# Hippogriff/prifit

Hardware: AMD Instinct MI355X
Metric: shapes/sec (fwd+bwd) B=24x2048 pts, PointNet++-MSG+ellipsoid fit (higher is better)
Workload: dtype f32; 1 GPU; configs[2]: PointNet++-MSG + mean-shift(10 it, <=25 clusters) + ellipsoid fit + convex loss, B=24x2048 per GPU, fwd+bwd+Adam; global_batch=24, points=2048, parallelism=dp1, cloud=blobs, embedding=clustered, backbone_grad_param=sa1.conv_blocks.0.0.weight, launch=eager

## Files before the change

### include/prifit_hip.h

```cpp
#ifndef PRIFIT_HIP_H
#define PRIFIT_HIP_H

#include <stdint.h>

#ifdef __cplusplus
extern "C" {
#endif

#define PRIFIT_OK 0
#define PRIFIT_EINVAL (-1)
#define PRIFIT_ELAUNCH (-2)

#define PRIFIT_ABI_VERSION 700
int prifit_version(const char **arch);


int prifit_fps(const float *xyz, int B, int N, int npoint, const int64_t *start_idx,
               int64_t *out_idx, float *new_xyz, void *stream);

int prifit_ball_query(const float *xyz, const float *new_xyz, int B, int N, int S, int R,
                      const float *radius2, const int *nsample, void *const *out, int idx64,
                      void *stream);

int prifit_three_nn(const float *xyz1, const float *xyz2, int B, int N, int S, int32_t *idx,
                    float *dist, float *weight, void *stream);

int prifit_square_distance(const float *src, const float *dst, int B, int S, int N, float *out,
                           void *stream);


int prifit_group_gather(const float *feat, const float *xyz, const float *new_xyz,
                        const int32_t *idx, int B, int N, int S, int K, int C, int order,
                        int ld_out, float *out, void *stream);

int prifit_group_scatter_add(const float *gout, int ld_gout, int col0, const int32_t *idx, int B,
                             int N, int S, int K, int C, float *dfeat, void *stream);

int prifit_pack_cols(const float *w, int rows, int src_cols, const int32_t *map, int dst_cols, float *out, void *stream);
int prifit_unpack_cols(const float *g, int rows, int dst_cols, const int32_t *inv_off, const int32_t *inv_idx, int src_cols,
                       float *gw, void *stream);
int prifit_pack_cols_max_jobs(void);
int prifit_pack_cols_multi(int njobs, const float *const *w, const int32_t *rows, const int32_t *src_cols, const int32_t *const *map,
                           const int32_t *dst_cols, float *const *out, void *stream);
int prifit_unpack_cols_multi(int njobs, const float *const *g, const int32_t *rows, const int32_t *dst_cols, const int32_t *const *inv_off,
                             const int32_t *const *inv_idx, const int32_t *src_cols, float *const *gw, void *stream);

int prifit_three_interpolate(const float *points2, const int32_t *idx, const float *weight, int B,
                             int N, int S, int C, int ld_out, int col0, float *out, void *stream);

int prifit_three_interpolate_bwd(const float *gout, int ld_gout, int col0, const int32_t *idx,
                                 const float *weight, int B, int N, int S, int C, float *dpoints2,
                                 void *stream);
int prifit_fp_rows(const float *points2, const int32_t *idx, const float *weight, const float *points1, int B, int N, int S, int D2,
                   int D1, int kp, float *out, void *stream);


#define PRIFIT_GEMM_NT 0
#define PRIFIT_GEMM_NN 1
#define PRIFIT_GEMM_TN 2
#define PRIFIT_EPI_NONE 0
#define PRIFIT_EPI_CHORD 1
#define PRIFIT_EPI_MSKERNEL 2
#define PRIFIT_EPI_MSBWD 3

int prifit_gemm_f32(int layout, int M, int N, int K, const float *A, long long lda, long long strideA,
                    const float *B, long long ldb, long long strideB, float *C, long long ldc,
                    long long strideC, int batch, int splitk, const float *a_scale,
                    const float *a_shift, const float *b_scale, const float *b_shift,
                    const float *bias, long long bias_batch_stride, float *col_stats, int epilogue,
                    const float *epi_batch_scalar, const float *epi_aux, long long ld_aux,
                    long long stride_aux, const float *epi_row_add, float *a_rowsum, int accumulate, void *stream);

int prifit_chord_sym_f32(const float *A, long long lda, long long strideA, float *C, long long ldc, long long strideC,
                         int n, int K, int batch, unsigned long long *owner_key, void *stream);
int prifit_chord_sym_mask(const float *A, long long lda, long long strideA, const float *thr, uint32_t *mask, int n, int K, int batch,
                          unsigned long long *owner_key, void *stream);
int prifit_gram_sym_f32(const float *A, long long lda, long long strideA, float *C, long long ldc, long long strideC, int n, int K,
                        int batch, void *stream);

int prifit_gemm_pool_f32(int M, int N, int K, const float *A, long long lda, const float *W, long long ldb, float *Y,
                         long long ldc, const float *a_scale, const float *a_shift, const float *bias, float *col_stats,
                         float *cand, void *stream);
int prifit_gemm_pool_supported(int M, int N, int K);

int prifit_gemm_stream_f32(int layout, int M, int N, int K, const float *A, long long lda, const float *B,
                           long long ldb, float *C, long long ldc, const float *a_scale, const float *a_shift,
                           const float *bias, float *col_stats, void *stream);
int prifit_gemm_stream_supported(int layout, int M, int N, int K);
int prifit_gemm_stream_slabs(int M, int K);

int prifit_gemm_dual_nn_f32(int M, int N, int K1, int K2, const float *A1, const float *A2, long long lda,
                            long long strideA, const float *B1, const float *B2, long long ldb, long long strideB,
                            float *C, long long ldc, long long strideC, int batch, int splitk, int accumulate,
                            void *stream);

int prifit_gemm_dgrad_bnred_f32(int M, int N, int K, const float *dY, long long lda, const float *W, long long ldb,
                                float *G, long long ldc, const float *Yprev, long long ldy, const float *scale,
                                const float *shift, const float *mean, const float *invstd, float *red_slab, void *stream);
int prifit_slab_sum(const float *part, int nslab, long long n, float *out, void *stream);
int prifit_global_pool_winners_supported(int Cout, int Cin);
int prifit_global_pool_winners_f32(int Bs, int K, int Cout, int Cin, const int32_t *arg, const float *T, const float *W,
                                   long long ldw, const float *X, long long ldx, float *dX, long long lddx, float *dW,
                                   long long lddw, void *stream);

int prifit_gemm_stream_gather_f32(int M, int N, const int32_t *idx, const float *U, const float *Vc, int n_points, int n_centres,
                                  int rows_per_centre, const float *B, long long ldb, float *C, long long ldc,
                                  const float *a_scale, const float *a_shift, const float *bias, float *col_stats, void *stream);
int prifit_gemm_stream_bwd_gather_f32(long long P, int Cout, const float *G, const float *Y, const float *scale,
                                      const float *shift, const float *coef_a, const float *coef_b, const float *coef_d,
                                      const float *W, long long ldw, const int32_t *idx, const float *U, const float *Vc,
                                      int n_points, int n_centres, int rows_per_centre, const float *p_scale,
                                      const float *p_shift, const float *p_mean, const float *p_invstd, float *Gp, long long ldgp,
                                      float *red_slab, float *dW, long long lddw, float *workspace, void *stream);
int prifit_gemm_stream_pool_f32(int M, int N, int K, const float *A, long long lda, const float *B, long long ldb,
                                float *C, long long ldc, const float *a_scale, const float *a_shift, const float *bias,
                                float *col_stats, float *cand, void *stream);
int prifit_pool_from_candidates(const float *cand, const float *scale, const float *shift, int G, int K, int C,
                                int rows_per_sample, float slope, float *out, long long ldo, int32_t *arg, float *ystar,
                                void *stream);

int prifit_gemm_stream_dgrad_f32(int M, int N, int K, const float *dY, long long lda, const float *W, long long ldb,
                                 float *G, long long ldc, const float *Yprev, long long ldy, const float *scale,
                                 const float *shift, const float *mean, const float *invstd, float *red_slab, void *stream);

int prifit_pool_bwd_table(const float *gp, long long ldgp, const float *Y, long long ldy, const int32_t *arg,
                          const float *scale, const float *shift, const float *coef_a, int G, int K, int C, float slope,
                          float *T, void *stream);
int prifit_gemm_stream_dgrad_pool_f32(int M, int N, int K, const float *Y, long long lda, const float *W, long long ldb,
                                      float *G, long long ldc, const float *bias_dW, const int32_t *pool_arg,
                                      const float *pool_T, const float *coef_b, int pool_K, const float *Yprev,
                                      long long ldy, const float *scale, const float *shift, const float *mean,
                                      const float *invstd, float *red_slab, void *stream);
int prifit_gemm_stream_tn_pool_f32(int Mo, int No, long long P, const float *Y, long long ldy, const float *A,
                                   long long lda, float *out, long long ldo, const float *b_scale,
                                   const float *b_shift, const int32_t *pool_arg, const float *pool_T,
                                   const float *coef_b, const float *coef_d, int pool_K, float *workspace,
                                   void *stream);

int prifit_gemm_stream_tn_bn_f32(int Mo, int No, long long P, const float *G, const float *Y, long long ldy, const float *A,
                                 long long lda, float *out, long long ldo, const float *b_scale, const float *b_shift,
                                 const float *scale, const float *shift, const float *coef_a, const float *coef_b,
                                 const float *coef_d, float *workspace, void *stream);
int prifit_gemm_stream_dgrad_bn_f32(int M, int N, int K, const float *Gin, const float *Y, long long lda, const float *W,
                                    long long ldb, float *G, long long ldc, const float *scale_l, const float *shift_l,
                                    const float *coef_a, const float *coef_b, const float *coef_d, const float *Yprev,
                                    long long ldy, const float *scale, const float *shift, const float *mean,
                                    const float *invstd, float *red_slab, void *stream);
int prifit_gemm_stream_tn_f32(int Mo, int No, long long P, const float *G, long long ldg, const float *A,
                              long long lda, float *out, long long ldo, const float *b_scale,
                              const float *b_shift, float *workspace, void *stream);
long long prifit_gemm_stream_tn_workspace(int Mo, int No, long long P);
int prifit_gemm_stream_tn_supported(int Mo, int No, long long P);

int prifit_gemm_tile_m(int N);
// ... 326 lines not shown
```

### prifit_amd/csrc/gemm.hip

```cpp
#include <stdlib.h>

#include <type_traits>

#include "common.h"

typedef float f32x16 __attribute__((ext_vector_type(16)));

enum { LAY_NT = 0, LAY_NN = 1, LAY_TN = 2 };
enum { EPI_NONE = 0, EPI_CHORD = 1, EPI_MSKERNEL = 2, EPI_MSBWD = 3, EPI_BNRED = 4 };

struct GemmArgs {
    const float *A, *B;
    float *C;
    int M, N, K;
    long long lda, ldb, ldc;
    long long sA, sB, sC;
    int batch, splitk;
    const float *a_scale, *a_shift;
    const float *b_scale, *b_shift;
    const float *bias;
    long long bias_stride;
    float *stats;
    int epi;
    const float *epi_batch_scalar;
    const float *aux;
    const float *row_add;
    float *a_rowsum;
    long long ldaux, sAux;
    const float *red_scale, *red_shift, *red_mean, *red_invstd;
    long long dA2, dB2;
    int kswitch;
    int accumulate;
    int vecA, vecB;
    int ntiles;
    float *cand;
};

#ifndef GEMM_W8
#define GEMM_W8 6
#endif
constexpr int BK = 32;
constexpr int PAD = 4;

__device__ __forceinline__ float4 ld4(const float *p) { return *reinterpret_cast<const float4 *>(p); }

template <int ROWS, bool KC, bool VEC, bool AFF, int NTH>
struct TileLoader {
    static constexpr int NV = ROWS * BK / 4 / NTH;
    static_assert(NV * NTH * 4 == ROWS * BK, "tile must divide evenly over the threads");
    float4 v[NV];
    const float *ptr[NV];
    int klo[NV];
    int c0[NV];
    unsigned okmask[NV];
    long long step;
    int K, R, cclamp;

    __device__ __forceinline__ void init(const float *__restrict__ base, long long ld, int r0, int R_, int K_)
    {
        K = K_; R = R_;
        step = KC ? (long long)BK : (long long)BK * ld;
#pragma unroll
        for (int p = 0; p < NV; ++p) {
            const int id = threadIdx.x + NTH * p;
            if (KC) {
                const int gr = r0 + id / (BK / 4);
                klo[p] = (id % (BK / 4)) * 4;
                okmask[p] = gr < R ? 0xFu : 0u;
                ptr[p] = base + (long long)(gr < R ? gr : 0) * ld + (klo[p] < K ? klo[p] : 0);
                c0[p] = 0;
            } else {
                klo[p] = id / (ROWS / 4);
                const int gr = r0 + (id % (ROWS / 4)) * 4;
                unsigned m = 0;
#pragma unroll
                for (int j = 0; j < 4; ++j) m |= (gr + j < R) ? (1u << j) : 0u;
                okmask[p] = m;
                c0[p] = m ? gr : 0;
                ptr[p] = base + (long long)klo[p] * ld + c0[p];
            }
        }
    }

    int kload;
// ... 163 lines not shown
    int klo[NV], c0[NV];
    __amdgpu_buffer_rsrc_t rs;
    const float *base;
    int step4, K, kload;

    __device__ __forceinline__ void init(const float *__restrict__ b, long long ld, int r0, int R, int K_)
    {
        K = K_;
        base = b;
        rs = __builtin_amdgcn_make_buffer_rsrc(const_cast<float *>(b), 0, 0x7ffffffc, 0x00020000);
        step4 = KC ? BK * 4 : (int)(BK * ld * 4);
#pragma unroll
        for (int p = 0; p < NV; ++p) {
            const int id = threadIdx.x + NTH * p;
            if (KC) {
                const int row = r0 + id / (BK / 4);
                klo[p] = (id % (BK / 4)) * 4;
                c0[p] = 0;
                voff[p] = row < R ? (int)(((long long)row * ld + klo[p]) * 4) : OOBV;
            } else {
                klo[p] = id / (ROWS / 4);
                c0[p] = r0 + (id % (ROWS / 4)) * 4;
                voff[p] = c0[p] < R ? (int)(((long long)klo[p] * ld + c0[p]) * 4) : OOBV;
                if (c0[p] >= R) c0[p] = 0;
            }
        }
    }
    __device__ __forceinline__ void load(int k0, const float *__restrict__, const float *__restrict__) { load(k0); }
    __device__ __forceinline__ void shift(long long delta)
    {
        base += delta;
        rs = __builtin_amdgcn_make_buffer_rsrc(const_cast<float *>(base), 0, 0x7ffffffc, 0x00020000);
    }
    __device__ __forceinline__ void load(int k0)
    {
        kload = k0;
        const int soff = (k0 / BK) * step4;
        if (k0 + BK <= K) {
#pragma unroll
            for (int p = 0; p < NV; ++p) {
                const f32x4v t = __builtin_bit_cast(f32x4v, __builtin_amdgcn_raw_buffer_load_b128(rs, voff[p], soff, 0));
                v[p] = make_float4(t.x, t.y, t.z, t.w);
            }
        } else {
#pragma unroll
            for (int p = 0; p < NV; ++p) {
                const int vo = k0 + klo[p] < K ? voff[p] : OOBV;
                const f32x4v t = __builtin_bit_cast(f32x4v, __builtin_amdgcn_raw_buffer_load_b128(rs, vo, soff, 0));
                v[p] = make_float4(t.x, t.y, t.z, t.w);
            }
        }
    }
    __device__ __forceinline__ void finish(const float *__restrict__ scale, const float *__restrict__ shift)
    {
        if (!AFF) return;
#pragma unroll
        for (int p = 0; p < NV; ++p) {
            const int gk = kload + klo[p];
            const bool ok = voff[p] != OOBV && gk < K;
            const int cc = KC ? (gk < K ? gk : 0) : c0[p];
            const float4 s = ld4(scale + cc), t = ld4(shift + cc);
            float4 x = v[p];
            x.x = fmaxf(fmaf(x.x, s.x, t.x), 0.f); x.y = fmaxf(fmaf(x.y, s.y, t.y), 0.f);
            x.z = fmaxf(fmaf(x.z, s.z, t.z), 0.f); x.w = fmaxf(fmaf(x.w, s.w, t.w), 0.f);
            v[p] = ok ? x : make_float4(0.f, 0.f, 0.f, 0.f);
        }
    }
    __device__ __forceinline__ void store(float *__restrict__ lds) const
    {
#pragma unroll
        for (int p = 0; p < NV; ++p) {
            const int id = threadIdx.x + NTH * p;
            if (KC) {
                const int row = id / (BK / 4), kk = (id % (BK / 4)) * 4;
                *reinterpret_cast<float4 *>(lds + row * (BK + PAD) + kk) = v[p];
            } else {
                const int kk = id / (ROWS / 4), row = (id % (ROWS / 4)) * 4;
                *reinterpret_cast<float4 *>(lds + kk * (ROWS + PAD) + row) = v[p];
            }
        }
    }
};

template <int ROWS, bool KC>
__device__ __forceinline__ float4 read_frag(const float *__restrict__ lds, int row, int g, int h)
{
    if (KC) return *reinterpret_cast<const float4 *>(lds + row * (BK + PAD) + g * 8 + h * 4);
    const float *p = lds + (g * 8 + h * 4) * (ROWS + PAD) + row;
    return make_float4(p[0], p[ROWS + PAD], p[2 * (ROWS + PAD)], p[3 * (ROWS + PAD)]);
}

template <int RA, bool AKC, int RB, bool BKC, int TN>
__device__ __forceinline__ void mma_ktile(const float *__restrict__ As, const float *__restrict__ Bs, int arow, int bcol, int lh,
                                          f32x16 (&acc)[TN], int ngk = BK / 8, int nbv = TN)
{
    float4 fa[2], fb[2][TN];
    fa[0] = read_frag<RA, AKC>(As, arow, 0, lh);
#pragma unroll
    for (int b = 0; b < TN; ++b)
        if (b < nbv) fb[0][b] = read_frag<RB, BKC>(Bs, bcol + 32 * b, 0, lh);
#pragma unroll
    for (int gk = 0; gk < BK / 8; ++gk) {
        if (gk > 0 && gk >= ngk) break;
        if (gk + 1 < BK / 8) {
            fa[(gk + 1) & 1] = read_frag<RA, AKC>(As, arow, gk + 1, lh);
#pragma unroll
            for (int b = 0; b < TN; ++b)
                if (b < nbv) fb[(gk + 1) & 1][b] = read_frag<RB, BKC>(Bs, bcol + 32 * b, gk + 1, lh);
        }
        __builtin_amdgcn_sched_barrier(0);
        const float4 a = fa[gk & 1];
#pragma unroll
        for (int b = 0; b < TN; ++b) {
            if (b >= nbv) continue;
            const float4 w = fb[gk & 1][b];
            acc[b] = __builtin_amdgcn_mfma_f32_32x32x2f32(a.x, w.x, acc[b], 0, 0, 0);
            acc[b] = __builtin_amdgcn_mfma_f32_32x32x2f32(a.y, w.y, acc[b], 0, 0, 0);
            acc[b] = __builtin_amdgcn_mfma_f32_32x32x2f32(a.z, w.z, acc[b], 0, 0, 0);
            acc[b] = __builtin_amdgcn_mfma_f32_32x32x2f32(a.w, w.w, acc[b], 0, 0, 0);
        }
        __builtin_amdgcn_sched_barrier(0);
    }
}

template <bool C, class A, class B> struct pick { typedef A type; };
template <class A, class B> struct pick<false, A, B> { typedef B type; };

template <int BM, int BN, int WM, int WN, int LAY, bool VA, bool VB, bool FA, bool FB, bool EX = false>
__global__ __launch_bounds__((BM / WM) * (BN / WN) * 64, ((BM / WM) * (BN / WN) == 8 ? GEMM_W8 : 4)) void gemm_kernel(const GemmArgs g)
{
    constexpr int NTH = (BM / WM) * (BN / WN) * 64;
    constexpr bool A_KC = (LAY != LAY_TN);
    constexpr bool B_KC = (LAY == LAY_NT);
    constexpr int TM = WM / 32, TN = WN / 32;
    constexpr int WAVES_N = BN / WN;
    static_assert(NTH == 256 || NTH == 512, "4 or 8 waves per block");
    constexpr int SZA = A_KC ? BM * (BK + PAD) : BK * (BM + PAD);
    constexpr int SZB = B_KC ? BN * (BK + PAD) : BK * (BN + PAD);
    __shared__ __attribute__((aligned(16))) float lds[2 * (SZA + SZB)];

    const int tilesN = (g.N + BN - 1) / BN;
    const int nwg = gridDim.x;
    int L;
    {
        const int bid = blockIdx.x, xcd = bid & 7, pos = bid >> 3, q = nwg >> 3, r = nwg & 7;
        L = (xcd < r ? xcd * (q + 1) : r * (q + 1) + (xcd - r) * q) + pos;
    }
    const int tile_m = L / tilesN, tile_n = L - tile_m * tilesN;
    const int m0 = tile_m * BM, n0 = tile_n * BN;
    const int z = blockIdx.z / g.splitk, ks = blockIdx.z - z * g.splitk;

    const float *A = g.A + (long long)z * g.sA;
    const float *B = g.B + (long long)z * g.sB;
    float *C = g.C + (long long)z * g.sC;

    const int ktiles = (g.K + BK - 1) / BK;
    const int per = (ktiles + g.splitk - 1) / g.splitk;
    const int kt0 = ks * per, kt1 = min(ktiles, kt0 + per);

    const int wave = threadIdx.x >> 6, lane = threadIdx.x & 63;
    const int li = lane & 31, lh = lane >> 5;
    const int wm0 = (wave / WAVES_N) * WM, wn0 = (wave % WAVES_N) * WN;

    f32x16 acc[TM][TN];
#pragma unroll
    for (int a = 0; a < TM; ++a)
#pragma unroll
        for (int b = 0; b < TN; ++b)
#pragma unroll
            for (int r = 0; r < 16; ++r) acc[a][b][r] = 0.f;

    typename pick<EX, BufLoader<BM, A_KC, FA, NTH>, TileLoader<BM, A_KC, VA, FA, NTH>>::type la;
    typename pick<EX, BufLoader<BN, B_KC, FB, NTH>, TileLoader<BN, B_KC, VB, FB, NTH>>::type lb;
    la.init(A, g.lda, m0, g.M, g.K);
    lb.init(B, g.ldb, n0, g.N, g.K);
    constexpr int NVA = TileLoader<BM, A_KC, VA, FA, NTH>::NV;
    float rs[NVA];
#pragma unroll
    for (int p = 0; p < NVA; ++p) rs[p] = 0.f;
    const bool want_rowsum = !EX && A_KC && g.a_rowsum != nullptr && tile_n == 0;

    const int kswitch = g.kswitch ? g.kswitch : 0x7fffffff;
    if (kt0 >= kswitch) { la.shift(g.dA2); lb.shift(g.dB2); }
    if (kt0 < kt1) {
        la.load(kt0 * BK, g.a_scale, g.a_shift);
        lb.load(kt0 * BK, g.b_scale, g.b_shift);
        la.finish(g.a_scale, g.a_shift);
        lb.finish(g.b_scale, g.b_shift);
        la.store(lds);
        lb.store(lds + SZA);
        if (want_rowsum) {
// ... 496 lines not shown
        }
        if (okz) {
            const int r = threadIdx.x & (BM - 1), q = threadIdx.x >> 7;
            float rmin = INFINITY;
            int ridx = 0;
#pragma unroll 8
            for (int c = 32 * q; c < 32 * q + 32; ++c) {
                const float v = lds[c * TLD + r];
                if (v < rmin) { rmin = v; ridx = c; }
            }
            atomicMin(okz + m0 + r, ((unsigned long long)fkey(rmin) << 32) | (unsigned)(n0 + ridx));
        }
    }
}

template <bool FB>
__global__ __launch_bounds__(512) __attribute__((amdgpu_waves_per_eu(4, 4))) void gemm_tnsk_kernel(const GemmArgs g)
{
    constexpr int BM = 128, BN = 128, WM = 32, WN = 64, NTH = 512, TN = WN / 32;
    constexpr int SZA = BK * (BM + PAD), SZB = BK * (BN + PAD);
    __shared__ __attribute__((aligned(16))) float lds[2 * (SZA + SZB)];
    const int tilesN = (g.N + BN - 1) / BN;
    const int tile_m = blockIdx.x / tilesN, tile_n = blockIdx.x - tile_m * tilesN;
    const int m0 = tile_m * BM, n0 = tile_n * BN;
    const int ktiles = (g.K + BK - 1) / BK;
    const int per = (ktiles + g.splitk - 1) / g.splitk;
    const int kt0 = blockIdx.z * per, kt1 = min(ktiles, kt0 + per);
    if (kt0 >= kt1) return;
    const int wave = __builtin_amdgcn_readfirstlane(threadIdx.x >> 6), lane = threadIdx.x & 63;
    const int li = lane & 31, lh = lane >> 5;
    const int wm0 = (wave % (BM / WM)) * WM, wn0 = (wave / (BM / WM)) * WN;
    const int nbv = m0 + wm0 >= g.M ? 0 : min(TN, max(0, (g.N - n0 - wn0 + 31) >> 5));

    BufLoader<BM, false, false, NTH> la[2];
    BufLoader<BN, false, FB, NTH> lb[2];
#pragma unroll
    for (int i = 0; i < 2; ++i) { la[i].init(g.A, g.lda, m0, g.M, g.K); lb[i].init(g.B, g.ldb, n0, g.N, g.K); }
    la[0].load(kt0 * BK); lb[0].load(kt0 * BK);
    if (kt0 + 1 < kt1) { la[1].load((kt0 + 1) * BK); lb[1].load((kt0 + 1) * BK); }
    lb[0].finish(g.b_scale, g.b_shift);
    la[0].store(lds); lb[0].store(lds + SZA);
    __syncthreads();
    f32x16 acc[TN];
#pragma unroll
    for (int b = 0; b < TN; ++b)
#pragma unroll
        for (int r = 0; r < 16; ++r) acc[b][r] = 0.f;
    auto step = [&](int kt, auto par) {
        constexpr int S = decltype(par)::value;
        const float *As = lds + S * (SZA + SZB), *Bs = As + SZA;
        if (kt + 2 < kt1) { la[S].load((kt + 2) * BK); lb[S].load((kt + 2) * BK); }
        __builtin_amdgcn_sched_barrier(0);
        mma_ktile<BM, false, BN, false, TN>(As, Bs, wm0 + li, wn0 + li, lh, acc, BK / 8, nbv);
        if (kt + 1 < kt1) {
            float *An = lds + (S ^ 1) * (SZA + SZB);
            lb[S ^ 1].finish(g.b_scale, g.b_shift);
            la[S ^ 1].store(An); lb[S ^ 1].store(An + SZA);
        }
        __syncthreads();
    };
    int kt = kt0;
    for (; kt + 1 < kt1; kt += 2) {
        step(kt, std::integral_constant<int, 0>());
        step(kt + 1, std::integral_constant<int, 1>());
    }
    if (kt < kt1) step(kt, std::integral_constant<int, 0>());
    const int rbase = m0 + wm0 + 4 * lh;
#pragma unroll
    for (int b = 0; b < TN; ++b) {
        const int col = n0 + wn0 + 32 * b + li;
        if (col >= g.N) continue;
#pragma unroll
        for (int r = 0; r < 16; ++r) {
            const int row = rbase + (r & 3) + 8 * (r >> 2);
            if (row >= g.M) continue;
            float *dst = g.C + (long long)row * g.ldc + col;
            if (g.splitk > 1) unsafeAtomicAdd(dst, acc[b][r]);
            else if (g.accumulate) *dst += acc[b][r];
            else *dst = acc[b][r];
        }
    }
}

static bool launch_tnsk(const GemmArgs &g, hipStream_t st)
{
    if (g.batch != 1 || g.a_scale || g.bias || g.stats || g.epi != EPI_NONE || g.a_rowsum || g.kswitch ||
        !(g.vecA && g.vecB) || (g.M & 3) || (g.N & 3) || (g.splitk > 1 && !g.accumulate) || g.splitk > 65535)
        return false;
    const long long lim = 0x7ff00000LL;
    if ((long long)g.K * g.lda * 4 >= lim || (long long)g.K * g.ldb * 4 >= lim) return false;
    const dim3 grid(((g.M + 127) / 128) * ((g.N + 127) / 128), 1, g.splitk), block(512);
    if (g.b_scale) hipLaunchKernelGGL((gemm_tnsk_kernel<true>), grid, block, 0, st, g);
    else hipLaunchKernelGGL((gemm_tnsk_kernel<false>), grid, block, 0, st, g);
    return true;
}

static bool launch_persistent(const GemmArgs &g_, int lay, hipStream_t st, float *want_cand = nullptr, bool dry = false)
{
    GemmArgs g = g_;
    if (lay == LAY_TN || g.batch != 1 || g.splitk != 1 || g.accumulate || g.a_rowsum || g.kswitch ||
        g.b_scale || !(g.epi == EPI_NONE || g.epi == EPI_BNRED) || !(g.vecA && g.vecB) || (g.K & 3) || (lay == LAY_NN && (g.N & 3)))
        return false;
    const long long lim = 0x7ff00000LL;
    if ((long long)g.M * g.lda * 4 >= lim || (long long)(lay == LAY_NT ? g.N : g.K) * g.ldb * 4 >= lim ||
        (long long)g.M * g.ldc * 4 >= lim || (g.epi == EPI_BNRED && (long long)g.M * g.ldaux * 4 >= lim))
        return false;
    g.ntiles = ((g.M + 127) / 128) * ((g.N + 127) / 128);
    const int slots = 512;
    if (g.ntiles <= slots) return false;
    if (dry) return lay == LAY_NT && g.epi == EPI_NONE && g.a_scale;
    const dim3 grid(slots), block(512);
    if (lay == LAY_NT) {
        if (g.epi != EPI_NONE) return false;
        if (want_cand) {
            g.cand = want_cand;
            if (g.a_scale) hipLaunchKernelGGL((gemm_pers_kernel<LAY_NT, true, false, true>), grid, block, 0, st, g);
            else hipLaunchKernelGGL((gemm_pers_kernel<LAY_NT, false, false, true>), grid, block, 0, st, g);
        } else if (g.a_scale) hipLaunchKernelGGL((gemm_pers_kernel<LAY_NT, true, false>), grid, block, 0, st, g);
        else hipLaunchKernelGGL((gemm_pers_kernel<LAY_NT, false, false>), grid, block, 0, st, g);
    } else {
        if (want_cand) return false;
        if (g.a_scale) return false;
        if (g.epi == EPI_BNRED) hipLaunchKernelGGL((gemm_pers_kernel<LAY_NN, false, true>), grid, block, 0, st, g);
        else hipLaunchKernelGGL((gemm_pers_kernel<LAY_NN, false, false>), grid, block, 0, st, g);
    }
    return true;
}

__global__ __launch_bounds__(512, 4) void gemm_dual_sk_kernel(const GemmArgs g)
{
    constexpr int BM = 128, BN = 128, WN = 64, NTH = 512, TN = 2, WAVES_N = 2;
    constexpr int SZA = BM * (BK + PAD), SZB = BK * (BN + PAD);
    __shared__ __attribute__((aligned(16))) float lds[2 * (SZA + SZB)];
    const int tilesM = g.M / BM;
    const int ktiles = g.K / BK;
    const long long total = (long long)g.batch * tilesM * ktiles;
    int u = (int)(total * blockIdx.x / gridDim.x);
    const int uend = (int)(total * (blockIdx.x + 1) / gridDim.x);
    const int wave = threadIdx.x >> 6, lane = threadIdx.x & 63;
    const int li = lane & 31, lh = lane >> 5;
    const int wm0 = (wave / WAVES_N) * 32, wn0 = (wave % WAVES_N) * WN;
    const int kswitch = g.kswitch ? g.kswitch : 0x7fffffff;

    while (u < uend) {
        const int t = u / ktiles;
        const int kt0 = u - t * ktiles, kt1 = min(ktiles, kt0 + (uend - u));
        const int z = t / tilesM, tile_m = t - z * tilesM;
        const int m0 = tile_m * BM;
        const float *A = g.A + (long long)z * g.sA;
        const float *B = g.B + (long long)z * g.sB;
        float *C = g.C + (long long)z * g.sC;

        f32x16 acc[TN];
#pragma unroll
        for (int b = 0; b < TN; ++b)
#pragma unroll
            for (int r = 0; r < 16; ++r) acc[b][r] = 0.f;
        ExactLoader<BM, true, false, NTH> la;
        ExactLoader<BN, false, false, NTH> lb;
        la.init(A, g.lda, m0, g.M, g.K);
        lb.init(B, g.ldb, 0, g.N, g.K);
        if (kt0 >= kswitch) { la.shift(g.dA2); lb.shift(g.dB2); }
        la.load(kt0 * BK, nullptr, nullptr);
        lb.load(kt0 * BK, nullptr, nullptr);
        la.store(lds);
        lb.store(lds + SZA);
        __syncthreads();
        for (int kt = kt0; kt < kt1; ++kt) {
            const int stage = (kt - kt0) & 1;
            const float *As = lds + stage * (SZA + SZB), *Bs = As + SZA;
            const bool more = kt + 1 < kt1;
            if (more) {
                if (kt + 1 == kswitch) { la.shift(g.dA2); lb.shift(g.dB2); }
                la.load((kt + 1) * BK, nullptr, nullptr);
                lb.load((kt + 1) * BK, nullptr, nullptr);
// ... 16 lines not shown
        }
        u += kt1 - kt0;
    }
}

template <int BM, int BN, int WM, int WN, int LAY, bool VEC>
static void launch_aff(const GemmArgs &g, dim3 grid, hipStream_t st)
{
    const dim3 block((BM / WM) * (BN / WN) * 64);
    const long long spanA = (LAY == LAY_TN ? (long long)g.K * g.lda : (long long)g.M * g.lda) * 4;
    const long long spanB = (LAY == LAY_NT ? (long long)g.N * g.ldb : (long long)g.K * g.ldb) * 4;
    const bool exact = VEC && !g.a_rowsum && spanA < 0x7ff00000LL && spanB < 0x7ff00000LL;
    if (exact) {
        if (g.a_scale) hipLaunchKernelGGL((gemm_kernel<BM, BN, WM, WN, LAY, true, true, true, false, true>), grid, block, 0, st, g);
        else if (g.b_scale) hipLaunchKernelGGL((gemm_kernel<BM, BN, WM, WN, LAY, true, true, false, true, true>), grid, block, 0, st, g);
        else hipLaunchKernelGGL((gemm_kernel<BM, BN, WM, WN, LAY, true, true, false, false, true>), grid, block, 0, st, g);
        return;
    }
    if (g.a_scale) hipLaunchKernelGGL((gemm_kernel<BM, BN, WM, WN, LAY, VEC, VEC, true, false>), grid, block, 0, st, g);
    else if (g.b_scale) hipLaunchKernelGGL((gemm_kernel<BM, BN, WM, WN, LAY, VEC, VEC, false, true>), grid, block, 0, st, g);
    else hipLaunchKernelGGL((gemm_kernel<BM, BN, WM, WN, LAY, VEC, VEC, false, false>), grid, block, 0, st, g);
}

template <int BM, int BN, int WM, int WN>
static int launch_cfg(const GemmArgs &g, int lay, hipStream_t st)
{
    const int tilesM = (g.M + BM - 1) / BM, tilesN = (g.N + BN - 1) / BN;
    dim3 grid(tilesM * tilesN, 1, g.batch * g.splitk);
    const bool vec = g.vecA && g.vecB;
    if (g.a_scale && g.b_scale) return PRIFIT_EINVAL;
    switch (lay) {
        case LAY_NT:
            if (vec) launch_aff<BM, BN, WM, WN, LAY_NT, true>(g, grid, st);
            else launch_aff<BM, BN, WM, WN, LAY_NT, false>(g, grid, st);
            break;
        case LAY_NN:
            if (vec) launch_aff<BM, BN, WM, WN, LAY_NN, true>(g, grid, st);
            else launch_aff<BM, BN, WM, WN, LAY_NN, false>(g, grid, st);
            break;
        default:
            if (vec) launch_aff<BM, BN, WM, WN, LAY_TN, true>(g, grid, st);
            else launch_aff<BM, BN, WM, WN, LAY_TN, false>(g, grid, st);
            break;
    }
    return prifit_check_launch();
}

static inline bool aligned16(const void *p) { return ((uintptr_t)p & 15) == 0; }

static inline bool small_tiles(int M, int N, int batch, int splitk)
{
    const long long wgs = (long long)((M + 127) / 128) * ((N + 127) / 128) * batch * splitk;
    return wgs < (splitk > 1 ? 160 : 520) && M > 64 && N > 32;
}

static int dispatch(GemmArgs &g, int layout, void *stream)
{
    const int M = g.M, N = g.N, K = g.K;
    const int extA = layout == LAY_TN ? M : K, extB = layout == LAY_NT ? K : N;
    g.vecA = aligned16(g.A) && (g.lda % 4 == 0) && (g.sA % 4 == 0) && (extA % 4 == 0);
    g.vecB = aligned16(g.B) && (g.ldb % 4 == 0) && (g.sB % 4 == 0) && (extB % 4 == 0);
    hipStream_t st = as_stream(stream);
    if (small_tiles(M, N, g.batch, g.splitk)) return launch_cfg<64, 64, 32, 32>(g, layout, st);
    if (N <= 32) return launch_cfg<128, 32, 32, 32>(g, layout, st);
    if (N <= 64) return launch_cfg<128, 64, 32, 64>(g, layout, st);
    if (N <= 96) return launch_cfg<128, 96, 32, 96>(g, layout, st);
    if (launch_persistent(g, layout, st)) return prifit_check_launch();
    if (layout == LAY_TN && launch_tnsk(g, st)) return prifit_check_launch();
    return launch_cfg<128, 128, 32, 64>(g, layout, st);
}

extern "C" {

#ifdef PERS_STAMPS
int prifit_debug_pers_ktail(int on)
{
    return hipMemcpyToSymbol(HIP_SYMBOL(g_pers_ktail), &on, sizeof(int)) == hipSuccess ? 0 : -1;
}
int prifit_debug_pers_stamps(unsigned long long *host, int n)
{
    return hipMemcpyFromSymbol(host, HIP_SYMBOL(g_pers_stamps), sizeof(unsigned long long) * (size_t)n) == hipSuccess ? 0 : -1;
}
#endif

int prifit_gemm_tile_m(int N)
{
    (void)N;
    return 128;
}

int prifit_gemm_stats_tile_m(int M, int N)
{
    return small_tiles(M, N, 1, 1) ? 64 : 128;
}

int prifit_gemm_f32(int layout, int M, int N, int K, const float *A, long long lda, long long strideA,
                    const float *B, long long ldb, long long strideB, float *C, long long ldc,
                    long long strideC, int batch, int splitk, const float *a_scale, const float *a_shift,
                    const float *b_scale, const float *b_shift, const float *bias, long long bias_batch_stride,
                    float *col_stats, int epilogue, const float *epi_batch_scalar, const float *epi_aux, long long ld_aux,
                    long long stride_aux, const float *epi_row_add, float *a_rowsum, int accumulate, void *stream)
{
    if (!A || !B || !C || M <= 0 || N <= 0 || K <= 0 || batch <= 0 || splitk <= 0 || layout < 0 || layout > 2 ||
        (epilogue != 100 && (epilogue < 0 || epilogue > 3)) || (epilogue >= EPI_MSKERNEL && !epi_batch_scalar) ||
        (epilogue == EPI_MSBWD && !epi_aux) || (splitk > 1 && !accumulate) ||
        ((a_scale == nullptr) != (a_shift == nullptr)) || ((b_scale == nullptr) != (b_shift == nullptr)) ||
        (col_stats && (batch != 1 || splitk != 1)) || (epilogue != EPI_NONE && epilogue != 100 && splitk != 1) || (long long)batch * splitk > 65535)
        return PRIFIT_EINVAL;
    GemmArgs g;
    g.A = A; g.B = B; g.C = C; g.M = M; g.N = N; g.K = K;
    g.lda = lda; g.ldb = ldb; g.ldc = ldc; g.sA = strideA; g.sB = strideB; g.sC = strideC;
    g.batch = batch; g.splitk = splitk;
    g.a_scale = a_scale; g.a_shift = a_shift; g.b_scale = b_scale; g.b_shift = b_shift;
    g.bias = bias; g.bias_stride = bias_batch_stride; g.stats = col_stats; g.epi = epilogue; g.epi_batch_scalar = epi_batch_scalar;
    g.accumulate = accumulate; g.aux = epi_aux; g.ldaux = ld_aux; g.sAux = stride_aux;
    g.row_add = epi_row_add; g.a_rowsum = a_rowsum;
    g.red_scale = g.red_shift = g.red_mean = g.red_invstd = nullptr;
    g.dA2 = g.dB2 = 0; g.kswitch = 0;
    if (a_rowsum && (layout == LAY_TN || splitk != 1)) return PRIFIT_EINVAL;
    return dispatch(g, layout, stream);
}

int prifit_gemm_dual_nn_f32(int M, int N, int K1, int K2, const float *A1, const float *A2, long long lda,
                            long long strideA, const float *B1, const float *B2, long long ldb, long long strideB,
                            float *C, long long ldc, long long strideC, int batch, int splitk, int accumulate,
                            void *stream)
{
    if (!A1 || !A2 || !B1 || !B2 || !C || M <= 0 || N <= 0 || K1 <= 0 || K2 <= 0 || (K1 % BK) || batch <= 0 ||
        splitk <= 0 || (splitk > 1 && !accumulate) || (long long)batch * splitk > 65535 || lda < K1 || lda < K2 ||
        ldb < N || ldc < N)
        return PRIFIT_EINVAL;
    if ((((uintptr_t)A1 ^ (uintptr_t)A2) | ((uintptr_t)B1 ^ (uintptr_t)B2)) & 15) return PRIFIT_EINVAL;
    GemmArgs g;
    g.A = A1; g.B = B1; g.C = C; g.M = M; g.N = N; g.K = K1 + K2;
    g.lda = lda; g.ldb = ldb; g.ldc = ldc; g.sA = strideA; g.sB = strideB; g.sC = strideC;
    g.batch = batch; g.splitk = splitk;
    g.a_scale = g.a_shift = g.b_scale = g.b_shift = nullptr;
    g.bias = nullptr; g.bias_stride = 0; g.stats = nullptr; g.epi = EPI_NONE; g.epi_batch_scalar = nullptr;
    g.accumulate = accumulate; g.aux = nullptr; g.ldaux = 0; g.sAux = 0; g.row_add = nullptr; g.a_rowsum = nullptr;
    g.red_scale = g.red_shift = g.red_mean = g.red_invstd = nullptr;
    g.dA2 = (A2 - A1) - (long long)K1;
    g.dB2 = (B2 - B1) - (long long)K1 * ldb;
    g.kswitch = K1 / BK;
    if (accumulate && N == 128 && M % 128 == 0 && K1 == K2 && aligned16(A1) && aligned16(B1) && (lda % 4 == 0) &&
        (ldb % 4 == 0) && (strideA % 4 == 0) && (strideB % 4 == 0) && (long long)M * lda * 4 < 0x7ff00000LL &&
        (long long)(K1 + K2) * ldb * 4 < 0x7ff00000LL) {
        static const int slots = [] {
            int dev = 0;
            hipDeviceProp_t p;
            if (hipGetDevice(&dev) != hipSuccess || hipGetDeviceProperties(&p, dev) != hipSuccess) return 512;
            return 2 * p.multiProcessorCount;
        }();
        const long long total = (long long)batch * (M / 128) * ((K1 + K2) / BK);
        const int grid = (int)(total < slots ? total : slots);
        hipLaunchKernelGGL(gemm_dual_sk_kernel, dim3(grid), dim3(512), 0, as_stream(stream), g);
        return prifit_check_launch();
    }
    return dispatch(g, LAY_NN, stream);
}

int prifit_gemm_dgrad_bnred_f32(int M, int N, int K, const float *dY, long long lda, const float *W, long long ldb,
                                float *G, long long ldc, const float *Yprev, long long ldy, const float *scale,
                                const float *shift, const float *mean, const float *invstd, float *red_slab, void *stream)
{
    if (!dY || !W || !G || !Yprev || !scale || !shift || !mean || !invstd || !red_slab || M <= 0 || N <= 0 || K <= 0 ||
        lda < K || ldb < N || ldc < N || ldy < N)
// ... 89 lines not shown
```

Measured before the change: 1640 shapes/s.

## Add multi-stage LDS ring pipeline for split-K TN GEMM using buffer-to-LDS loads

Adds a new split-K TN GEMM kernel that loads A and B tiles straight into LDS through buffer_load_lds. A multi-stage ring buffer overlaps the global loads with the MFMA work, and the optional ReLU/BN affine on B is applied in place in LDS. The 2-stage, KT=32 variant becomes the default route for TN split-K GEMMs (weight gradients); an env var and an API can select the old register kernel or 3- and 4-stage variants. It aims to hide global memory latency better than the register-staged kernel, at the cost of more LDS use and fixed occupancy.

```diff
diff --git a/include/prifit_hip.h b/include/prifit_hip.h
--- a/include/prifit_hip.h
+++ b/include/prifit_hip.h
@@ -11,7 +11,7 @@
 #define PRIFIT_EINVAL (-1)
 #define PRIFIT_ELAUNCH (-2)
 
-#define PRIFIT_ABI_VERSION 700
+#define PRIFIT_ABI_VERSION 701
 int prifit_version(const char **arch);
 
 
@@ -70,6 +70,9 @@
                     const float *bias, long long bias_batch_stride, float *col_stats, int epilogue,
                     const float *epi_batch_scalar, const float *epi_aux, long long ld_aux,
                     long long stride_aux, const float *epi_row_add, float *a_rowsum, int accumulate, void *stream);
+
+int prifit_gemm_tn_route(int M, int N, int K, long long lda, long long ldb, int splitk, int b_affine, int accumulate);
+int prifit_gemm_tnsk_mode(int mode);
 
 int prifit_chord_sym_f32(const float *A, long long lda, long long strideA, float *C, long long ldc, long long strideC,
                          int n, int K, int batch, unsigned long long *owner_key, void *stream);
diff --git a/prifit_amd/csrc/gemm.hip b/prifit_amd/csrc/gemm.hip
--- a/prifit_amd/csrc/gemm.hip
+++ b/prifit_amd/csrc/gemm.hip
@@ -1,5 +1,6 @@
 #include <stdlib.h>
 
+#include <string>
 #include <type_traits>
 
 #include "common.h"
@@ -329,31 +330,31 @@
     }
 };
 
-template <int ROWS, bool KC>
+template <int ROWS, bool KC, int PD = PAD>
 __device__ __forceinline__ float4 read_frag(const float *__restrict__ lds, int row, int g, int h)
 {
-    if (KC) return *reinterpret_cast<const float4 *>(lds + row * (BK + PAD) + g * 8 + h * 4);
-    const float *p = lds + (g * 8 + h * 4) * (ROWS + PAD) + row;
-    return make_float4(p[0], p[ROWS + PAD], p[2 * (ROWS + PAD)], p[3 * (ROWS + PAD)]);
-}
-
-template <int RA, bool AKC, int RB, bool BKC, int TN>
+    if (KC) return *reinterpret_cast<const float4 *>(lds + row * (BK + PD) + g * 8 + h * 4);
+    const float *p = lds + (g * 8 + h * 4) * (ROWS + PD) + row;
+    return make_float4(p[0], p[ROWS + PD], p[2 * (ROWS + PD)], p[3 * (ROWS + PD)]);
+}
+
+template <int RA, bool AKC, int RB, bool BKC, int TN, int PD = PAD, int NGK = BK / 8>
 __device__ __forceinline__ void mma_ktile(const float *__restrict__ As, const float *__restrict__ Bs, int arow, int bcol, int lh,
-                                          f32x16 (&acc)[TN], int ngk = BK / 8, int nbv = TN)
+                                          f32x16 (&acc)[TN], int ngk = NGK, int nbv = TN)
 {
     float4 fa[2], fb[2][TN];
-    fa[0] = read_frag<RA, AKC>(As, arow, 0, lh);
+    fa[0] = read_frag<RA, AKC, PD>(As, arow, 0, lh);
 #pragma unroll
     for (int b = 0; b < TN; ++b)
-        if (b < nbv) fb[0][b] = read_frag<RB, BKC>(Bs, bcol + 32 * b, 0, lh);
-#pragma unroll
-    for (int gk = 0; gk < BK / 8; ++gk) {
+        if (b < nbv) fb[0][b] = read_frag<RB, BKC, PD>(Bs, bcol + 32 * b, 0, lh);
+#pragma unroll
+    for (int gk = 0; gk < NGK; ++gk) {
         if (gk > 0 && gk >= ngk) break;
-        if (gk + 1 < BK / 8) {
-            fa[(gk + 1) & 1] = read_frag<RA, AKC>(As, arow, gk + 1, lh);
+        if (gk + 1 < NGK) {
+            fa[(gk + 1) & 1] = read_frag<RA, AKC, PD>(As, arow, gk + 1, lh);
 #pragma unroll
             for (int b = 0; b < TN; ++b)
-                if (b < nbv) fb[(gk + 1) & 1][b] = read_frag<RB, BKC>(Bs, bcol + 32 * b, gk + 1, lh);
+                if (b < nbv) fb[(gk + 1) & 1][b] = read_frag<RB, BKC, PD>(Bs, bcol + 32 * b, gk + 1, lh);
         }
         __builtin_amdgcn_sched_barrier(0);
         const float4 a = fa[gk & 1];
@@ -1016,15 +1017,163 @@
     }
 }
 
+__device__ __forceinline__ void relu_bn_in_place(float4 *__restrict__ q, const float4 s, const float4 t, bool ok)
+{
+    float4 x = *q;
+    x.x = fmaxf(fmaf(x.x, s.x, t.x), 0.f); x.y = fmaxf(fmaf(x.y, s.y, t.y), 0.f);
+    x.z = fmaxf(fmaf(x.z, s.z, t.z), 0.f); x.w = fmaxf(fmaf(x.w, s.w, t.w), 0.f);
+    *q = ok ? x : make_float4(0.f, 0.f, 0.f, 0.f);
+}
+
+__device__ __forceinline__ void load_lds16(__amdgpu_buffer_rsrc_t rs, float *dst, unsigned voff)
+{
+    __builtin_amdgcn_raw_ptr_buffer_load_lds(rs, (__attribute__((address_space(3))) void *)dst, 16, voff, 0, 0, 0);
+}
+
+template <bool FB, int S, int KT>
+__global__ __launch_bounds__(512) __attribute__((amdgpu_waves_per_eu(4, 4))) void gemm_tnsk_ring_kernel(const GemmArgs g)
+{
+    constexpr int BM = 128, BN = 128, WM = 32, WN = 64, NTH = 512, TN = WN / 32;
+    constexpr int SZ = KT * 128;
+    constexpr int NV = SZ / 4 / NTH;
+    constexpr int IPT = 2 * NV;
+    constexpr unsigned OOB = 0x80000000u;
+    static_assert(BK % KT == 0 && KT % 8 == 0 && NV >= 1 && S >= 2 && IPT * (S - 2) < 16, "ring shape");
+    __shared__ __attribute__((aligned(16))) float lds[S * 2 * SZ];
+    const int tilesN = (g.N + BN - 1) / BN;
+    const int tile_m = blockIdx.x / tilesN, tile_n = blockIdx.x - tile_m * tilesN;
+    const int m0 = tile_m * BM, n0 = tile_n * BN;
+    const int ktiles = (g.K + BK - 1) / BK;
+    const int per = (ktiles + g.splitk - 1) / g.splitk;
+    const int kt0 = blockIdx.z * per, kt1 = min(ktiles, kt0 + per);
+    if (kt0 >= kt1) return;
+    const int wave = __builtin_amdgcn_readfirstlane(threadIdx.x >> 6), lane = threadIdx.x & 63;
+    const int li = lane & 31, lh = lane >> 5;
+    const int wm0 = (wave % (BM / WM)) * WM, wn0 = (wave / (BM / WM)) * WN;
+    const int nbv = m0 + wm0 >= g.M ? 0 : min(TN, max(0, (g.N - n0 - wn0 + 31) >> 5));
+
+    const int kbeg = kt0 * BK, kend = min(kt1 * BK, g.K);
+    const int nt = (kt1 - kt0) * (BK / KT);
+    const __amdgpu_buffer_rsrc_t ars = __builtin_amdgcn_make_buffer_rsrc(const_cast<float *>(g.A), 0, (int)(kend * g.lda * 4), 0x00020000);
+    const __amdgpu_buffer_rsrc_t brs = __builtin_amdgcn_make_buffer_rsrc(const_cast<float *>(g.B), 0, (int)(kend * g.ldb * 4), 0x00020000);
+    const unsigned astep = (unsigned)(KT * g.lda * 4), bstep = (unsigned)(KT * g.ldb * 4);
+    unsigned aoff[NV], boff[NV];
+    int bk[NV];
+    float4 bs[NV], bt[NV];
+#pragma unroll
+    for (int p = 0; p < NV; ++p) {
+        const int id = threadIdx.x + NTH * p, kk = id >> 5, c = (id & 31) * 4;
+        aoff[p] = m0 + c < g.M ? (unsigned)(((kbeg + kk) * g.lda + m0 + c) * 4) : OOB;
+        boff[p] = n0 + c < g.N ? (unsigned)(((kbeg + kk) * g.ldb + n0 + c) * 4) : OOB;
+        bk[p] = kk;
+        if (FB) {
+            const int cc = n0 + c < g.N ? n0 + c : 0;
+            bs[p] = ld4(g.b_scale + cc); bt[p] = ld4(g.b_shift + cc);
+            asm volatile("" : "+v"(bs[p].x), "+v"(bs[p].y), "+v"(bs[p].z), "+v"(bs[p].w), "+v"(bt[p].x), "+v"(bt[p].y), "+v"(bt[p].z), "+v"(bt[p].w));
+        }
+    }
+    auto issue = [&](int j, int st) {
+        float *dst = lds + st * 2 * SZ + wave * 256;
+        const bool in = j < nt;
+#pragma unroll
+        for (int p = 0; p < NV; ++p)
+            load_lds16(ars, dst + p * NTH * 4, in ? aoff[p] + (unsigned)j * astep : OOB);
+#pragma unroll
+        for (int p = 0; p < NV; ++p)
+            load_lds16(brs, dst + SZ + p * NTH * 4, in ? boff[p] + (unsigned)j * bstep : OOB);
+    };
+#pragma unroll
+    for (int j = 0; j < S - 1; ++j) issue(j, j);
+    f32x16 acc[TN];
+#pragma unroll
+    for (int b = 0; b < TN; ++b)
+#pragma unroll
+        for (int r = 0; r < 16; ++r) acc[b][r] = 0.f;
+    auto ring = [&](auto nb) {
+        constexpr int NB = decltype(nb)::value;
+        int st = 0;
+        for (int j = 0; j < nt; ++j) {
+            asm volatile("s_waitcnt vmcnt(%0)" ::"n"(IPT * (S - 2)) : "memory");
+            float *As = lds + st * 2 * SZ, *Bs = As + SZ;
+            if (FB) {
+#pragma unroll
+                for (int p = 0; p < NV; ++p) {
+                    const bool ok = boff[p] != OOB && kbeg + j * KT + bk[p] < g.K;
+                    relu_bn_in_place(reinterpret_cast<float4 *>(Bs + (threadIdx.x + NTH * p) * 4), bs[p], bt[p], ok);
+                }
+                asm volatile("s_waitcnt lgkmcnt(0)" ::: "memory");
+            }
+            __builtin_amdgcn_s_barrier();
+            issue(j + S - 1, st == 0 ? S - 1 : st - 1);
+            __builtin_amdgcn_sched_barrier(0);
+            if constexpr (NB > 0)
+                mma_ktile<BM, false, BN, false, NB, 0, KT / 8>(As, Bs, wm0 + li, wn0 + li, lh, reinterpret_cast<f32x16(&)[NB]>(acc));
+            st = st + 1 == S ? 0 : st + 1;
+        }
+    };
+    if (nbv == TN) ring(std::integral_constant<int, TN>());
+    else if (nbv == 1) ring(std::integral_constant<int, 1>());
+    else ring(std::integral_constant<int, 0>());
+    asm volatile("s_waitcnt vmcnt(0)" ::: "memory");
+    const int rbase = m0 + wm0 + 4 * lh;
+#pragma unroll
+    for (int b = 0; b < TN; ++b) {
+        const int col = n0 + wn0 + 32 * b + li;
+        if (col >= g.N) continue;
+#pragma unroll
+        for (int r = 0; r < 16; ++r) {
+            const int row = rbase + (r & 3) + 8 * (r >> 2);
+            if (row >= g.M) continue;
+            float *dst = g.C + (long long)row * g.ldc + col;
+            if (g.splitk > 1) unsafeAtomicAdd(dst, acc[b][r]);
+            else if (g.accumulate) *dst += acc[b][r];
+            else *dst = acc[b][r];
+        }
+    }
+}
+
+enum { TNSK_OFF = 0, TNSK_REG = 1, TNSK_RING2 = 2, TNSK_RING3 = 3, TNSK_RING4 = 4, TNSK_DEFAULT = TNSK_RING2 };
+static int g_tnsk_override = -1;
+static int tnsk_mode()
+{
+    static const int env = [] {
+        const char *e = getenv("PRIFIT_GEMM_TNSK");
+        if (!e) return (int)TNSK_DEFAULT;
+        const std::string v(e);
+        return v == "0" ? (int)TNSK_OFF : v == "reg" ? (int)TNSK_REG : v == "s2" ? (int)TNSK_RING2 : v == "s3" ? (int)TNSK_RING3 :
+               v == "s4" ? (int)TNSK_RING4 : (int)TNSK_DEFAULT;
+    }();
+    return g_tnsk_override >= 0 ? g_tnsk_override : env;
+}
+
+static int tnsk_route(const GemmArgs &g)
+{
+    const int mode = tnsk_mode();
+    if (mode == TNSK_OFF || g.batch != 1 || g.a_scale || g.bias || g.stats || g.epi != EPI_NONE || g.a_rowsum || g.kswitch ||
+        !(g.vecA && g.vecB) || (g.M & 3) || (g.N & 3) || (g.splitk > 1 && !g.accumulate) || g.splitk > 65535)
+        return TNSK_OFF;
+    const long long lim = 0x7ff00000LL;
+    if ((long long)g.K * g.lda * 4 >= lim || (long long)g.K * g.ldb * 4 >= lim) return TNSK_OFF;
+    if (mode != TNSK_REG && ((long long)(g.K + BK) * g.lda * 4 >= lim || (long long)(g.K + BK) * g.ldb * 4 >= lim)) return TNSK_REG;
+    return mode;
+}
+
+template <int S, int KT>
+static void launch_tnsk_ring(const GemmArgs &g, dim3 grid, hipStream_t st)
+{
+    if (g.b_scale) hipLaunchKernelGGL((gemm_tnsk_ring_kernel<true, S, KT>), grid, dim3(512), 0, st, g);
+    else hipLaunchKernelGGL((gemm_tnsk_ring_kernel<false, S, KT>), grid, dim3(512), 0, st, g);
+}
+
 static bool launch_tnsk(const GemmArgs &g, hipStream_t st)
 {
-    if (g.batch != 1 || g.a_scale || g.bias || g.stats || g.epi != EPI_NONE || g.a_rowsum || g.kswitch ||
-        !(g.vecA && g.vecB) || (g.M & 3) || (g.N & 3) || (g.splitk > 1 && !g.accumulate) || g.splitk > 65535)
-        return false;
-    const long long lim = 0x7ff00000LL;
-    if ((long long)g.K * g.lda * 4 >= lim || (long long)g.K * g.ldb * 4 >= lim) return false;
+    const int arm = tnsk_route(g);
+    if (arm == TNSK_OFF) return false;
     const dim3 grid(((g.M + 127) / 128) * ((g.N + 127) / 128), 1, g.splitk), block(512);
-    if (g.b_scale) hipLaunchKernelGGL((gemm_tnsk_kernel<true>), grid, block, 0, st, g);
+    if (arm == TNSK_RING2) launch_tnsk_ring<2, 32>(g, grid, st);
+    else if (arm == TNSK_RING3) launch_tnsk_ring<3, 16>(g, grid, st);
+    else if (arm == TNSK_RING4) launch_tnsk_ring<4, 16>(g, grid, st);
+    else if (g.b_scale) hipLaunchKernelGGL((gemm_tnsk_kernel<true>), grid, block, 0, st, g);
     else hipLaunchKernelGGL((gemm_tnsk_kernel<false>), grid, block, 0, st, g);
     return true;
 }
@@ -1207,6 +1356,27 @@
     return hipMemcpyFromSymbol(host, HIP_SYMBOL(g_pers_stamps), sizeof(unsigned long long) * (size_t)n) == hipSuccess ? 0 : -1;
 }
 #endif
+
+int prifit_gemm_tnsk_mode(int mode)
+{
+    if (mode < -1 || mode > TNSK_RING4) return PRIFIT_EINVAL;
+    g_tnsk_override = mode;
+    return 0;
+}
+
+int prifit_gemm_tn_route(int M, int N, int K, long long lda, long long ldb, int splitk, int b_affine, int accumulate)
+{
+    if (M <= 0 || N <= 0 || K <= 0 || splitk <= 0) return -1;
+    static const float one = 1.f;
+    GemmArgs g = {};
+    g.M = M; g.N = N; g.K = K; g.lda = lda; g.ldb = ldb; g.batch = 1; g.splitk = splitk; g.accumulate = accumulate;
+    g.epi = EPI_NONE;
+    g.b_scale = g.b_shift = b_affine ? &one : nullptr;
+    g.vecA = (lda % 4 == 0) && (M % 4 == 0);
+    g.vecB = (ldb % 4 == 0) && (N % 4 == 0);
+    if (small_tiles(M, N, 1, splitk) || N <= 96) return TNSK_OFF;
+    return tnsk_route(g);
+}
 
 int prifit_gemm_tile_m(int N)
 {
```

Result: no change. 1651 shapes/s, median of 6 (+0.7%).
